# Sue1347/SMSUT-MedicalImgSegmentation

Hardware: AMD Instinct MI355X
Metric: slices/sec uganConsisTrainer step @256x256 (higher is better)
Workload: dtype f32

## Files before the change

smsut-medicalimgsegmentation_amd/csrc/conv1x1.hip:

```cpp
#include "common.h"

namespace {

typedef float f32x4 __attribute__((ext_vector_type(4)));
constexpr int TPB = 256;

__device__ __forceinline__ f32x4 mfma16(float a, float b, f32x4 c) {
  return __builtin_amdgcn_mfma_f32_16x16x4f32(a, b, c, 0, 0, 0);
}

template <int MR, int NR, bool DUAL = false, bool PS = false>
__global__ void __launch_bounds__(TPB)
conv1x1_fwd(const float* __restrict__ x, const float* __restrict__ w, float* __restrict__ y, float* __restrict__ stats,
            int64_t P, int HW, int Kdim, int Ndim, int transposed, float* __restrict__ y2 = nullptr, int split = 0,
            const float* __restrict__ x2 = nullptr, int ca = 0, int ps_w = 0) {
  constexpr int CO_T = 16 * NR;
  extern __shared__ float w_s[];
  const int tid = threadIdx.x, lane = tid & 63, wave = tid >> 6;
  const int lm = lane & 15, kq = lane >> 4;
  const int co0 = blockIdx.y * CO_T;
  const int chunks = (Kdim + 15) / 16;
  for (int u = tid; u < chunks * 4 * CO_T; u += TPB) {
    const int n = u % CO_T;
    const int kg = (u / CO_T) * 4;
    const int ng = co0 + n;
    float4 v = make_float4(0.f, 0.f, 0.f, 0.f);
    if (ng < Ndim && kg < Kdim) {
      if constexpr (PS) {
        const int cout = Ndim >> 2, tap = ng / cout;
        const float* p = w + ((size_t)tap * Kdim + kg) * cout + (ng - tap * cout);
        v.x = p[0]; v.y = p[cout]; v.z = p[2 * (size_t)cout]; v.w = p[3 * (size_t)cout];
      } else if (!transposed) {
        const float* p = w + (size_t)kg * Ndim + ng;
        v.x = p[0]; v.y = p[Ndim]; v.z = p[2 * (size_t)Ndim]; v.w = p[3 * (size_t)Ndim];
      } else {
        v = *(const float4*)(w + (size_t)ng * Kdim + kg);
      }
    }
    *(float4*)(w_s + (size_t)u * 4) = v;
  }
  __syncthreads();

  const int64_t p0 = ((int64_t)blockIdx.x * 4 + wave) * (16 * MR);
  if (p0 >= P) return;
  f32x4 acc[MR][NR];
#pragma unroll
  for (int i = 0; i < MR; ++i)
#pragma unroll
    for (int j = 0; j < NR; ++j) acc[i][j] = (f32x4){0.f, 0.f, 0.f, 0.f};
  const float* xp[MR];
  const float* xq[MR];
  bool pok[MR];
  const int sa = DUAL ? ca : Kdim;
#pragma unroll
  for (int i = 0; i < MR; ++i) {
    const int64_t p = p0 + i * 16 + lm;
    pok[i] = p < P;
    xp[i] = x + (size_t)(pok[i] ? p : 0) * sa + 4 * kq;
    xq[i] = DUAL ? x2 + (size_t)(pok[i] ? p : 0) * (Kdim - ca) + 4 * kq - ca : xp[i];
  }
  for (int c = 0; c < chunks; ++c) {
    const bool kok = c * 16 + 4 * kq < Kdim;
    const bool second = DUAL && c * 16 >= ca;
    f32x4 a[MR], b[NR];
#pragma unroll
    for (int i = 0; i < MR; ++i)
      a[i] = (pok[i] && kok) ? *(const f32x4*)((second ? xq[i] : xp[i]) + c * 16) : (f32x4){0.f, 0.f, 0.f, 0.f};
#pragma unroll
    for (int j = 0; j < NR; ++j) b[j] = *(const f32x4*)(w_s + ((size_t)(c * 4 + kq) * CO_T + j * 16 + lm) * 4);
#pragma unroll
    for (int s = 0; s < 4; ++s)
#pragma unroll
      for (int i = 0; i < MR; ++i)
#pragma unroll
        for (int j = 0; j < NR; ++j) acc[i][j] = mfma16(a[i][s], b[j][s], acc[i][j]);
  }
#pragma unroll
  for (int j = 0; j < NR; ++j) {
    const int co = co0 + j * 16 + lm;
    const bool hi = y2 && co0 + j * 16 >= split;
    float* const yo = hi ? y2 : y;
    const int os = !y2 ? Ndim : (hi ? Ndim - split : split);
    const int oc = hi ? co - split : co;
    float s1 = 0.f, s2 = 0.f;
    if constexpr (PS) {
      const int cout = Ndim >> 2, tap = (co0 + j * 16) / cout, cc = co - tap * cout;
      const int W2 = 2 * ps_w;
#pragma unroll
      for (int i = 0; i < MR; ++i)
#pragma unroll
        for (int r = 0; r < 4; ++r) {
          const int64_t p = p0 + i * 16 + 4 * kq + r;
          if (p < P && co < Ndim) {
            const int row = (int)p / ps_w;
            const int wx = (int)p - row * ps_w;
            y[((size_t)(2 * row + (tap >> 1)) * W2 + 2 * wx + (tap & 1)) * cout + cc] = acc[i][j][r];
          }
        }
      continue;
    }
#pragma unroll
    for (int i = 0; i < MR; ++i)
#pragma unroll
      for (int r = 0; r < 4; ++r) {
        const int64_t p = p0 + i * 16 + 4 * kq + r;
        if (p < P && co < Ndim) {
          const float v = acc[i][j][r];
          yo[(size_t)p * os + oc] = v;
          s1 += v; s2 += v * v;
        }
      }
    if (stats) {
      s1 += __shfl_xor(s1, 16, 64); s2 += __shfl_xor(s2, 16, 64);
      s1 += __shfl_xor(s1, 32, 64); s2 += __shfl_xor(s2, 32, 64);
      if (kq == 0 && co < Ndim) {
        const int tiles = HW / (16 * MR);
        const int64_t n_img = p0 / HW;
        const int tile = (int)((p0 % HW) / (16 * MR));
        float* o = stats + (((size_t)n_img * tiles + tile) * Ndim + co) * 2;
        o[0] = s1; o[1] = s2;
      }
    }
  }
}

#ifndef W1_UNR
#define W1_UNR 4
#endif
template <int CIT, int COT, bool PS = false>
__global__ void __launch_bounds__(TPB)
conv1x1_wgrad(const float* __restrict__ x, const float* __restrict__ gy, float* __restrict__ part, int64_t P, int Cin,
              int Cout, int64_t pix_per_split, const float* __restrict__ x2 = nullptr, int ca = 0, int ps_w = 0) {
  __shared__ float red[CIT * COT * 64 * 4];
  const int tid = threadIdx.x, lane = tid & 63, wave = tid >> 6;
  const int lm = lane & 15, kq = lane >> 4;
  const int ci0 = blockIdx.y * (16 * CIT), co0 = blockIdx.z * (16 * COT);
  const int64_t pb = (int64_t)blockIdx.x * pix_per_split;
  const int64_t pe = min(pb + pix_per_split, P);
  f32x4 acc[CIT][COT];
#pragma unroll
  for (int i = 0; i < CIT; ++i)
#pragma unroll
    for (int j = 0; j < COT; ++j) acc[i][j] = (f32x4){0.f, 0.f, 0.f, 0.f};
  bool iok[CIT], jok[COT];
#pragma unroll
  for (int i = 0; i < CIT; ++i) iok[i] = ci0 + i * 16 + lm < Cin;
#pragma unroll
  for (int j = 0; j < COT; ++j) jok[j] = co0 + j * 16 + lm < Cout;
  CatSrc xs[CIT];
#pragma unroll
  for (int i = 0; i < CIT; ++i) xs[i] = cat_src(x, x2, Cin, ca, ci0 + i * 16);
  const float* gb = gy + co0 + lm;
  [[maybe_unused]] const int cout = Cout >> 2;
  [[maybe_unused]] int ps_tap[COT], ps_cc[COT];
  if constexpr (PS) {
#pragma unroll
    for (int j = 0; j < COT; ++j) { ps_tap[j] = (co0 + j * 16) / cout; ps_cc[j] = co0 + j * 16 - ps_tap[j] * cout + lm; }
  }
  constexpr int UNR = W1_UNR;
  for (int64_t p0 = pb + 4 * wave + kq; p0 - kq < pe; p0 += 16 * UNR) {
    float a[UNR][CIT], b[UNR][COT];
#pragma unroll
    for (int u = 0; u < UNR; ++u) {
      const int64_t p = p0 + 16 * u;
      const bool ok = p < pe;
#pragma unroll
      for (int i = 0; i < CIT; ++i) a[u][i] = (ok && iok[i]) ? xs[i].p[(size_t)p * xs[i].stride + ci0 + i * 16 + lm - xs[i].coff] : 0.f;
      if constexpr (PS) {
        const int row = (int)p / ps_w;
        const int wx = (int)p - row * ps_w;
#pragma unroll
        for (int j = 0; j < COT; ++j)
          b[u][j] = (ok && jok[j]) ? gy[((size_t)(2 * row + (ps_tap[j] >> 1)) * (2 * ps_w) + 2 * wx + (ps_tap[j] & 1)) * cout + ps_cc[j]] : 0.f;
      } else {
#pragma unroll
        for (int j = 0; j < COT; ++j) b[u][j] = (ok && jok[j]) ? gb[(size_t)p * Cout + j * 16] : 0.f;
      }
    }
#pragma unroll
    for (int u = 0; u < UNR; ++u)
#pragma unroll
      for (int i = 0; i < CIT; ++i)
#pragma unroll
        for (int j = 0; j < COT; ++j) acc[i][j] = mfma16(a[u][i], b[u][j], acc[i][j]);
  }
  for (int src = 1; src < 4; ++src) {
    __syncthreads();
    if (wave == src) {
#pragma unroll
      for (int i = 0; i < CIT; ++i)
#pragma unroll
        for (int j = 0; j < COT; ++j) *(f32x4*)(red + ((size_t)(i * COT + j) * 64 + lane) * 4) = acc[i][j];
    }
    __syncthreads();
    if (wave == 0) {
#pragma unroll
      for (int i = 0; i < CIT; ++i)
#pragma unroll
        for (int j = 0; j < COT; ++j) acc[i][j] += *(const f32x4*)(red + ((size_t)(i * COT + j) * 64 + lane) * 4);
    }
  }
  if (wave == 0) {
    float* out = part + (size_t)blockIdx.x * Cin * Cout;
#pragma unroll
    for (int i = 0; i < CIT; ++i)
#pragma unroll
      for (int j = 0; j < COT; ++j) {
        const int co = co0 + j * 16 + lm;
#pragma unroll
        for (int r = 0; r < 4; ++r) {
          const int ci = ci0 + i * 16 + 4 * kq + r;
          if constexpr (PS) {
            if (ci < Cin && co < Cout) out[((size_t)ps_tap[j] * Cin + ci) * cout + ps_cc[j]] = acc[i][j][r];
          } else if (ci < Cin && co < Cout) out[(size_t)ci * Cout + co] = acc[i][j][r];
        }
      }
  }
}

__global__ void __launch_bounds__(TPB)
sum_parts(const float* __restrict__ part, float* __restrict__ out, int wsize, int splits) {
  __shared__ float4 sm[TPB];
  const int col = threadIdx.x & 15, sl = threadIdx.x >> 4;
  const int e = (blockIdx.x * 16 + col) * 4;
  float4 t0 = make_float4(0.f, 0.f, 0.f, 0.f), t1 = t0, t2 = t0, t3 = t0;
  if (e < wsize) {
    int c = sl;
    for (; c + 48 < splits; c += 64) {
      const float4 v0 = *(const float4*)(part + (size_t)c * wsize + e);
      const float4 v1 = *(const float4*)(part + (size_t)(c + 16) * wsize + e);
      const float4 v2 = *(const float4*)(part + (size_t)(c + 32) * wsize + e);
      const float4 v3 = *(const float4*)(part + (size_t)(c + 48) * wsize + e);
      t0.x += v0.x; t0.y += v0.y; t0.z += v0.z; t0.w += v0.w; t1.x += v1.x; t1.y += v1.y; t1.z += v1.z; t1.w += v1.w;
      t2.x += v2.x; t2.y += v2.y; t2.z += v2.z; t2.w += v2.w; t3.x += v3.x; t3.y += v3.y; t3.z += v3.z; t3.w += v3.w;
    }
    for (; c < splits; c += 16) {
      const float4 v = *(const float4*)(part + (size_t)c * wsize + e);
      t0.x += v.x; t0.y += v.y; t0.z += v.z; t0.w += v.w;
    }
  }
  sm[threadIdx.x] = make_float4((t0.x + t1.x) + (t2.x + t3.x), (t0.y + t1.y) + (t2.y + t3.y), (t0.z + t1.z) + (t2.z + t3.z),
                                (t0.w + t1.w) + (t2.w + t3.w));
  __syncthreads();
  if (sl == 0 && e < wsize) {
    float4 t = sm[col];
    for (int l = 1; l < 16; ++l) { const float4 v = sm[l * 16 + col]; t.x += v.x; t.y += v.y; t.z += v.z; t.w += v.w; }
    *(float4*)(out + e) = t;
  }
}

struct Plan1 { int splits; int64_t pps; };
inline Plan1 plan_wgrad1(int64_t P, int Cin, int Cout, int cit, int cot) {
  const int slabs = ((Cin + 16 * cit - 1) / (16 * cit)) * ((Cout + 16 * cot - 1) / (16 * cot));
  int64_t want = (1024 + slabs - 1) / slabs;
  const int64_t maxs = P / 256 > 0 ? P / 256 : 1;
  if (want > maxs) want = maxs;
  if (want < 1) want = 1;
  Plan1 p;
  p.pps = ((P + want - 1) / want + 15) / 16 * 16;
  p.splits = (int)((P + p.pps - 1) / p.pps);
  return p;
}


constexpr int THIN_MAX = 8;

template <int CI>
__global__ void __launch_bounds__(TPB)
thin1x1_dgrad(const float* __restrict__ gy, const float* __restrict__ w, float* __restrict__ gx, int64_t P, int CO) {
  constexpr int Q = CI / 4;
  __shared__ float wt[THIN_MAX * CI];
  for (int u = threadIdx.x; u < THIN_MAX * CI; u += TPB) {
    const int k = u / CI, ci = u % CI;
    wt[u] = k < CO ? w[ci * CO + k] : 0.f;
  }
  __syncthreads();
  const int64_t total = P * Q;
  for (int64_t i = (int64_t)blockIdx.x * TPB + threadIdx.x; i < total; i += (int64_t)gridDim.x * TPB) {
    const int c4 = (int)(i % Q);
    const int64_t px = i / Q;
    float g[THIN_MAX];
#pragma unroll
    for (int k = 0; k < THIN_MAX; ++k) g[k] = k < CO ? gy[px * CO + k] : 0.f;
    f32x4 o = {0.f, 0.f, 0.f, 0.f};
#pragma unroll
    for (int k = 0; k < THIN_MAX; ++k) o += g[k] * *(const f32x4*)(wt + k * CI + c4 * 4);
    *(f32x4*)(gx + i * 4) = o;
  }
}

template <int CI>
__global__ void __launch_bounds__(TPB)
thin1x1_wgrad(const float* __restrict__ x, const float* __restrict__ gy, float* __restrict__ part, int64_t P, int CO) {
  constexpr int Q = CI / 4;
  static_assert(Q <= 64 && (Q & (Q - 1)) == 0, "lanes sharing a channel group sit Q apart inside a wave");
  __shared__ float sm[4 * Q * 4 * THIN_MAX];
  f32x4 acc[THIN_MAX];
#pragma unroll
  for (int k = 0; k < THIN_MAX; ++k) acc[k] = (f32x4){0.f, 0.f, 0.f, 0.f};
  const int64_t total = P * Q;
  const int64_t stride = (int64_t)gridDim.x * TPB;
  auto step = [&](int64_t i) {
    const int64_t px = i / Q;
    const f32x4 xv = *(const f32x4*)(x + i * 4);
#pragma unroll
    for (int k = 0; k < THIN_MAX; ++k) {
      const float g = k < CO ? gy[px * CO + k] : 0.f;
      acc[k] += g * xv;
    }
  };
  int64_t i = (int64_t)blockIdx.x * TPB + threadIdx.x;
  for (; i + stride < total; i += 2 * stride) { step(i); step(i + stride); }
  for (; i < total; i += stride) step(i);
  for (int off = Q; off < 64; off <<= 1) {
#pragma unroll
    for (int k = 0; k < THIN_MAX; ++k)
#pragma unroll
      for (int j = 0; j < 4; ++j) acc[k][j] += __shfl_xor(acc[k][j], off, 64);
  }
  const int lane = threadIdx.x & 63, wv = threadIdx.x >> 6;
  if (lane < Q) {
#pragma unroll
    for (int k = 0; k < THIN_MAX; ++k) *(f32x4*)(sm + ((wv * Q + lane) * THIN_MAX + k) * 4) = acc[k];
  }
  __syncthreads();
  if (threadIdx.x < Q) {
    const int c4 = threadIdx.x;
#pragma unroll
    for (int k = 0; k < THIN_MAX; ++k) {
      f32x4 t = *(const f32x4*)(sm + ((0 * Q + c4) * THIN_MAX + k) * 4);
#pragma unroll
      for (int w4 = 1; w4 < 4; ++w4) t += *(const f32x4*)(sm + ((w4 * Q + c4) * THIN_MAX + k) * 4);
#pragma unroll
      for (int j = 0; j < 4; ++j) part[((size_t)blockIdx.x * CI + c4 * 4 + j) * THIN_MAX + k] = t[j];
    }
  }
}

__global__ void __launch_bounds__(TPB)
thin1x1_wsum(const float* __restrict__ part, float* __restrict__ gw, int blocks, int CI, int CO) {
  const int lane = threadIdx.x & 63;
  const int col = blockIdx.x * 4 + (threadIdx.x >> 6);
  if (col >= CI * THIN_MAX / 4) return;
  f32x4 t = {0.f, 0.f, 0.f, 0.f};
  for (int b = lane; b < blocks; b += 64) t += *(const f32x4*)(part + ((size_t)b * CI * THIN_MAX) + col * 4);
  for (int off = 1; off < 64; off <<= 1)
#pragma unroll
    for (int j = 0; j < 4; ++j) t[j] += __shfl_xor(t[j], off, 64);
  if (lane == 0) {
    const int ci = col / 2, k0 = (col & 1) * 4;
#pragma unroll
    for (int j = 0; j < 4; ++j)
      if (k0 + j < CO) gw[ci * CO + k0 + j] = t[j];
  }
}

constexpr int THIN_WGRAD_BLOCKS = 1024;

}

extern "C" {

int smsut_conv1x1_supported(int Kdim, int Ndim) { return Kdim >= 4 && (Kdim % 4) == 0 && Kdim <= 512 && Ndim >= 1; }

int smsut_conv1x1_tiles(int N, int HW, int Ndim) {
  const int64_t P = (int64_t)N * HW;
  const int mr = (P / 256 >= 512) ? 4 : 1;
  (void)Ndim;
  return (HW % (16 * mr) == 0) ? HW / (16 * mr) : 0;
}

static int conv1x1_fwd_launch(const float* x, const float* w, float* y, float* stats, int N, int HW, int Kdim, int Ndim,
                              int transposed, void* stream, float* y2, int split, const float* x2 = nullptr, int ca = 0) {
  SMSUT_REQUIRE(x && w && y && N > 0 && HW > 0 && smsut_conv1x1_supported(Kdim, Ndim));
  SMSUT_REQUIRE(!y2 || (!stats && split > 0 && split < Ndim && split % 16 == 0));
  SMSUT_REQUIRE(!x2 || (!transposed && ca > 0 && ca < Kdim && ca % 16 == 0 && (Kdim - ca) % 4 == 0));
  const int64_t P = (int64_t)N * HW;
  const int mr = (P / 256 >= 512) ? 4 : 1;
  SMSUT_REQUIRE(!stats || HW % (16 * mr) == 0);
  const int nr = Ndim <= 16 ? 1 : 2;
  const int chunks = (Kdim + 15) / 16;
  const size_t sh = (size_t)chunks * 4 * 16 * nr * 4 * sizeof(float);
  dim3 grid((unsigned)cdiv64(P, 64 * mr), (Ndim + 16 * nr - 1) / (16 * nr));
  hipStream_t st = (hipStream_t)stream;
#define LAUNCH1X1(M, R)                                                                                                      \
  do {                                                                                                                       \
    if (x2) conv1x1_fwd<M, R, true><<<grid, TPB, sh, st>>>(x, w, y, stats, P, HW, Kdim, Ndim, transposed, y2, split, x2, ca); \
    else conv1x1_fwd<M, R, false><<<grid, TPB, sh, st>>>(x, w, y, stats, P, HW, Kdim, Ndim, transposed, y2, split, nullptr, 0); \
  } while (0)
  if (mr == 4 && nr == 2) LAUNCH1X1(4, 2);
  else if (mr == 4) LAUNCH1X1(4, 1);
  else if (nr == 2) LAUNCH1X1(1, 2);
  else LAUNCH1X1(1, 1);
#undef LAUNCH1X1
  SMSUT_LAUNCH_CHECK();
  return SMSUT_OK;
}

int smsut_conv1x1_fwd(const float* x, const float* w, float* y, float* stats, int N, int HW, int Kdim, int Ndim,
                      int transposed, void* stream) {
  return conv1x1_fwd_launch(x, w, y, stats, N, HW, Kdim, Ndim, transposed, stream, nullptr, 0);
}

int smsut_conv1x1_fwd_cat(const float* xa, const float* xb, int ca, const float* w, float* y, float* stats, int N, int HW,
                          int Kdim, int Ndim, void* stream) {
  SMSUT_REQUIRE(xb);
  return conv1x1_fwd_launch(xa, w, y, stats, N, HW, Kdim, Ndim, 0, stream, nullptr, 0, xb, ca);
}

int smsut_conv1x1_fwd_split(const float* x, const float* w, float* ya, float* yb, int split, int N, int HW, int Kdim,
                            int Ndim, int transposed, void* stream) {
  SMSUT_REQUIRE(yb);
  return conv1x1_fwd_launch(x, w, ya, nullptr, N, HW, Kdim, Ndim, transposed, stream, yb, split);
}

int smsut_convT2x2_ps_supported(int Cin, int Cout) {
  return Cout == 16 && Cin <= 256 && smsut_conv1x1_supported(Cin, 4 * Cout);
}

int smsut_convT2x2_fwd_ps(const float* x, const float* w, float* y, int N, int H, int W, int Cin, int Cout, void* stream) {
  SMSUT_REQUIRE(x && w && y && N > 0 && H > 0 && W > 0 && smsut_convT2x2_ps_supported(Cin, Cout));
  const int64_t P = (int64_t)N * H * W;
  SMSUT_REQUIRE(P * 4 * Cout < (1ll << 31));
  const int Nd = 4 * Cout;
  const int mr = (P / 256 >= 512) ? 4 : 1;
  const int nr = (Nd % 64 == 0) ? 4 : 2;
  const int chunks = (Cin + 15) / 16;
  const size_t sh = (size_t)chunks * 4 * 16 * nr * 4 * sizeof(float);
  dim3 grid((unsigned)cdiv64(P, 64 * mr), Nd / (16 * nr));
  hipStream_t st = (hipStream_t)stream;
#define PS_GO(M, R) conv1x1_fwd<M, R, false, true><<<grid, TPB, sh, st>>>(x, w, y, nullptr, P, H * W, Cin, Nd, 0, nullptr, 0, nullptr, 0, W)
  if (mr == 4 && nr == 4) PS_GO(4, 4);
  else if (mr == 4) PS_GO(4, 2);
  else if (nr == 4) PS_GO(1, 4);
  else PS_GO(1, 2);
#undef PS_GO
  SMSUT_LAUNCH_CHECK();
  return SMSUT_OK;
}

int64_t smsut_convT2x2_wgrad_ps_ws(int N, int H, int W, int Cin, int Cout) {
  const int cit = Cin > 16 ? 2 : 1;
  return (int64_t)plan_wgrad1((int64_t)N * H * W, Cin, 4 * Cout, cit, 2).splits * Cin * 4 * Cout;
}

int smsut_convT2x2_wgrad_ps(const float* x, const float* gy, float* gw, float* workspace, int N, int H, int W, int Cin,
                            int Cout, void* stream) {
  SMSUT_REQUIRE(x && gy && gw && workspace && N > 0 && H > 0 && W > 0 && smsut_convT2x2_ps_supported(Cin, Cout));
  const int64_t P = (int64_t)N * H * W;
  SMSUT_REQUIRE(P * 4 * Cout < (1ll << 31));
  const int Nd = 4 * Cout;
  const int cit = Cin > 16 ? 2 : 1;
  const Plan1 p = plan_wgrad1(P, Cin, Nd, cit, 2);
  dim3 grid(p.splits, (Cin + 16 * cit - 1) / (16 * cit), Nd / 32);
  hipStream_t st = (hipStream_t)stream;
  if (cit == 2) conv1x1_wgrad<2, 2, true><<<grid, TPB, 0, st>>>(x, gy, workspace, P, Cin, Nd, p.pps, nullptr, 0, W);
  else conv1x1_wgrad<1, 2, true><<<grid, TPB, 0, st>>>(x, gy, workspace, P, Cin, Nd, p.pps, nullptr, 0, W);
  const int wsize = Cin * Nd;
  sum_parts<<<(wsize + 63) / 64, TPB, 0, st>>>(workspace, gw, wsize, p.splits);
  SMSUT_LAUNCH_CHECK();
  return SMSUT_OK;
}

int64_t smsut_conv1x1_wgrad_ws(int N, int HW, int Cin, int Cout) {
  const int cit = Cin > 16 ? 2 : 1, cot = Cout > 16 ? 2 : 1;
  return (int64_t)plan_wgrad1((int64_t)N * HW, Cin, Cout, cit, cot).splits * Cin * Cout;
}

static int conv1x1_wgrad_launch(const float* x, const float* gy, float* gw, float* workspace, int N, int HW, int Cin,
                                int Cout, void* stream, const float* x2, int ca) {
  SMSUT_REQUIRE(x && gy && gw && workspace && N > 0 && HW > 0 && Cin > 0 && Cout > 0);
  SMSUT_REQUIRE(!x2 || (ca > 0 && ca < Cin && ca % 16 == 0));
  SMSUT_REQUIRE(((int64_t)Cin * Cout) % 4 == 0);
  const int64_t P = (int64_t)N * HW;
  const int cit = Cin > 16 ? 2 : 1, cot = Cout > 16 ? 2 : 1;
  const Plan1 p = plan_wgrad1(P, Cin, Cout, cit, cot);
  dim3 grid(p.splits, (Cin + 16 * cit - 1) / (16 * cit), (Cout + 16 * cot - 1) / (16 * cot));
  hipStream_t st = (hipStream_t)stream;
  if (cit == 2 && cot == 2) conv1x1_wgrad<2, 2><<<grid, TPB, 0, st>>>(x, gy, workspace, P, Cin, Cout, p.pps, x2, ca);
  else if (cit == 2) conv1x1_wgrad<2, 1><<<grid, TPB, 0, st>>>(x, gy, workspace, P, Cin, Cout, p.pps, x2, ca);
  else if (cot == 2) conv1x1_wgrad<1, 2><<<grid, TPB, 0, st>>>(x, gy, workspace, P, Cin, Cout, p.pps, x2, ca);
  else conv1x1_wgrad<1, 1><<<grid, TPB, 0, st>>>(x, gy, workspace, P, Cin, Cout, p.pps, x2, ca);
  const int wsize = Cin * Cout;
  sum_parts<<<(wsize + 63) / 64, TPB, 0, st>>>(workspace, gw, wsize, p.splits);
  SMSUT_LAUNCH_CHECK();
  return SMSUT_OK;
}

int smsut_conv1x1_wgrad(const float* x, const float* gy, float* gw, float* workspace, int N, int HW, int Cin, int Cout,
                        void* stream) {
  return conv1x1_wgrad_launch(x, gy, gw, workspace, N, HW, Cin, Cout, stream, nullptr, 0);
}

int smsut_conv1x1_wgrad_cat(const float* xa, const float* xb, int ca, const float* gy, float* gw, float* workspace, int N,
                            int HW, int Cin, int Cout, void* stream) {
  SMSUT_REQUIRE(xb);
  return conv1x1_wgrad_launch(xa, gy, gw, workspace, N, HW, Cin, Cout, stream, xb, ca);
}

int smsut_conv1x1_thin_supported(int Cin, int Cout) {
  return (Cin == 8 || Cin == 16 || Cin == 32 || Cin == 64) && Cout >= 1 && Cout <= THIN_MAX;
}

int smsut_conv1x1_thin_dgrad(const float* gy, const float* w, float* gx, int N, int HW, int Cin, int Cout, void* stream) {
  SMSUT_REQUIRE(gy && w && gx && N > 0 && HW > 0 && smsut_conv1x1_thin_supported(Cin, Cout));
  const int64_t P = (int64_t)N * HW;
  hipStream_t st = (hipStream_t)stream;
  const int grid = ew_grid(P * (Cin / 4));
  switch (Cin) {
    case 8: thin1x1_dgrad<8><<<grid, TPB, 0, st>>>(gy, w, gx, P, Cout); break;
    case 16: thin1x1_dgrad<16><<<grid, TPB, 0, st>>>(gy, w, gx, P, Cout); break;
    case 32: thin1x1_dgrad<32><<<grid, TPB, 0, st>>>(gy, w, gx, P, Cout); break;
    default: thin1x1_dgrad<64><<<grid, TPB, 0, st>>>(gy, w, gx, P, Cout); break;
  }
  SMSUT_LAUNCH_CHECK();
  return SMSUT_OK;
}

int64_t smsut_conv1x1_thin_wgrad_ws(int Cin) { return (int64_t)THIN_WGRAD_BLOCKS * Cin * THIN_MAX; }

int smsut_conv1x1_thin_wgrad(const float* x, const float* gy, float* gw, float* workspace, int N, int HW, int Cin,
                             int Cout, void* stream) {
  SMSUT_REQUIRE(x && gy && gw && workspace && N > 0 && HW > 0 && smsut_conv1x1_thin_supported(Cin, Cout));
  const int64_t P = (int64_t)N * HW;
  hipStream_t st = (hipStream_t)stream;
  int blocks = (int)cdiv64(P * (Cin / 4), 2 * TPB);
  if (blocks > THIN_WGRAD_BLOCKS) blocks = THIN_WGRAD_BLOCKS;
  switch (Cin) {
    case 8: thin1x1_wgrad<8><<<blocks, TPB, 0, st>>>(x, gy, workspace, P, Cout); break;
    case 16: thin1x1_wgrad<16><<<blocks, TPB, 0, st>>>(x, gy, workspace, P, Cout); break;
    case 32: thin1x1_wgrad<32><<<blocks, TPB, 0, st>>>(x, gy, workspace, P, Cout); break;
    default: thin1x1_wgrad<64><<<blocks, TPB, 0, st>>>(x, gy, workspace, P, Cout); break;
  }
  thin1x1_wsum<<<(Cin * THIN_MAX / 4 + 3) / 4, TPB, 0, st>>>(workspace, gw, blocks, Cin, Cout);
  SMSUT_LAUNCH_CHECK();
  return SMSUT_OK;
}

}
```

Baseline: 830.9.

## Make 1x1 conv forward persistent with prefetched inputs and LDS-staged vector stores

Turns the 1x1 conv forward kernel into a persistent grid. Each workgroup stages the weights into LDS once and then walks many pixel tiles, double-buffering the next group of input chunks in registers so the loads overlap the MFMA work. Output tiles are transposed through a small per-wave LDS exchange so they can be written as 16-byte vector stores instead of scalar strided stores. The weight staging loop is also unrolled. In exchange the kernel adds register pressure from the prefetch buffers and more template variants, and the occupancy-based grid cap may leave some CUs underused.

```diff
diff --git a/smsut-medicalimgsegmentation_amd/csrc/conv1x1.hip b/smsut-medicalimgsegmentation_amd/csrc/conv1x1.hip
--- a/smsut-medicalimgsegmentation_amd/csrc/conv1x1.hip
+++ b/smsut-medicalimgsegmentation_amd/csrc/conv1x1.hip
@@ -1,4 +1,5 @@
 #include "common.h"
+#include <type_traits>
 
 namespace {
 
@@ -9,119 +10,190 @@
   return __builtin_amdgcn_mfma_f32_16x16x4f32(a, b, c, 0, 0, 0);
 }
 
-template <int MR, int NR, bool DUAL = false, bool PS = false>
+#define FENCE1() do { asm volatile("" ::: "memory"); __builtin_amdgcn_sched_barrier(0); } while (0)
+
+#ifndef FWD1_WGS_PER_CU_MR1
+#define FWD1_WGS_PER_CU_MR1 4
+#endif
+#ifndef FWD1_WGS_PER_CU_MR4
+#define FWD1_WGS_PER_CU_MR4 2
+#endif
+constexpr int FWD1_AHEAD = 4;
+constexpr int FWD1_STAGE_UNR = 4;
+constexpr int XCH_STRIDE = 20;
+constexpr int XCH_FLOATS = 4 * 16 * XCH_STRIDE;
+
+template <int MR, int NR, int G, bool DUAL = false, bool PS = false>
 __global__ void __launch_bounds__(TPB)
 conv1x1_fwd(const float* __restrict__ x, const float* __restrict__ w, float* __restrict__ y, float* __restrict__ stats,
-            int64_t P, int HW, int Kdim, int Ndim, int transposed, float* __restrict__ y2 = nullptr, int split = 0,
+            int64_t P, int HW, int Kdim, int Ndim, int transposed, int xchg, float* __restrict__ y2 = nullptr, int split = 0,
             const float* __restrict__ x2 = nullptr, int ca = 0, int ps_w = 0) {
   constexpr int CO_T = 16 * NR;
-  extern __shared__ float w_s[];
+  extern __shared__ __attribute__((aligned(16))) float w_s[];
   const int tid = threadIdx.x, lane = tid & 63, wave = tid >> 6;
   const int lm = lane & 15, kq = lane >> 4;
   const int co0 = blockIdx.y * CO_T;
   const int chunks = (Kdim + 15) / 16;
-  for (int u = tid; u < chunks * 4 * CO_T; u += TPB) {
-    const int n = u % CO_T;
-    const int kg = (u / CO_T) * 4;
-    const int ng = co0 + n;
-    float4 v = make_float4(0.f, 0.f, 0.f, 0.f);
-    if (ng < Ndim && kg < Kdim) {
-      if constexpr (PS) {
-        const int cout = Ndim >> 2, tap = ng / cout;
-        const float* p = w + ((size_t)tap * Kdim + kg) * cout + (ng - tap * cout);
-        v.x = p[0]; v.y = p[cout]; v.z = p[2 * (size_t)cout]; v.w = p[3 * (size_t)cout];
-      } else if (!transposed) {
-        const float* p = w + (size_t)kg * Ndim + ng;
-        v.x = p[0]; v.y = p[Ndim]; v.z = p[2 * (size_t)Ndim]; v.w = p[3 * (size_t)Ndim];
-      } else {
-        v = *(const float4*)(w + (size_t)ng * Kdim + kg);
+  const int64_t ntiles = (P + 16 * MR - 1) / (16 * MR);
+  const int64_t tstride = (int64_t)gridDim.x * 4;
+  int64_t t = (int64_t)blockIdx.x * 4 + wave;
+  const int ngroups = (chunks + G - 1) / G;
+  int g = 0;
+  const int sa = DUAL ? ca : Kdim;
+  auto load = [&](f32x4 (&a)[G][MR], int64_t tile, int grp) {
+#pragma unroll
+    for (int i = 0; i < MR; ++i) {
+      const int64_t p = tile * (16 * MR) + i * 16 + lm;
+      const size_t pc = p < P ? (size_t)p : 0;
+      const float* xa = x + pc * sa;
+      [[maybe_unused]] const float* xb = DUAL ? x2 + pc * (Kdim - ca) : xa;
+#pragma unroll
+      for (int cc = 0; cc < G; ++cc) {
+        const int k = (grp * G + cc) * 16 + 4 * kq;
+        const bool second = DUAL && (grp * G + cc) * 16 >= ca;
+        const int off = k < Kdim ? (second ? k - ca : k) : 0;
+        a[cc][i] = *(const f32x4*)((second ? xb : xa) + off);
       }
     }
-    *(float4*)(w_s + (size_t)u * 4) = v;
-  }
+  };
+  f32x4 a0[G][MR], a1[G][MR];
+
+  const int units = chunks * 4 * CO_T;
+  auto stage = [&](auto tr_c) {
+    constexpr bool TR = decltype(tr_c)::value;
+    for (int u0 = tid; u0 < units; u0 += TPB * FWD1_STAGE_UNR) {
+      float4 v[FWD1_STAGE_UNR];
+#pragma unroll
+      for (int s = 0; s < FWD1_STAGE_UNR; ++s) {
+        const int u = u0 + s * TPB;
+        const int n = u % CO_T;
+        const int kg = (u / CO_T) * 4;
+        const int ng = co0 + n;
+        const bool ok = u < units && ng < Ndim && kg < Kdim;
+        if constexpr (PS) {
+          const int cout = Ndim >> 2, tap = ng / cout;
+          const float* p = ok ? w + ((size_t)tap * Kdim + kg) * cout + (ng - tap * cout) : w;
+          const size_t sw = ok ? cout : 0;
+          v[s] = make_float4(p[0], p[sw], p[2 * sw], p[3 * sw]);
+        } else if constexpr (!TR) {
+          const float* p = ok ? w + (size_t)kg * Ndim + ng : w;
+          const size_t sw = ok ? Ndim : 0;
+          v[s] = make_float4(p[0], p[sw], p[2 * sw], p[3 * sw]);
+        } else {
+          v[s] = *(const float4*)(ok ? w + (size_t)ng * Kdim + kg : w);
+        }
+        if (!ok) v[s] = make_float4(0.f, 0.f, 0.f, 0.f);
+      }
+#pragma unroll
+      for (int s = 0; s < FWD1_STAGE_UNR; ++s)
+        if (u0 + s * TPB < units) *(float4*)(w_s + (size_t)(u0 + s * TPB) * 4) = v[s];
+    }
+  };
+  if (PS || !transposed) stage(std::false_type{});
+  else stage(std::true_type{});
   __syncthreads();
 
-  const int64_t p0 = ((int64_t)blockIdx.x * 4 + wave) * (16 * MR);
-  if (p0 >= P) return;
+  if (t >= ntiles) return;
+  load(a0, t, 0);
   f32x4 acc[MR][NR];
 #pragma unroll
   for (int i = 0; i < MR; ++i)
 #pragma unroll
     for (int j = 0; j < NR; ++j) acc[i][j] = (f32x4){0.f, 0.f, 0.f, 0.f};
-  const float* xp[MR];
-  const float* xq[MR];
-  bool pok[MR];
-  const int sa = DUAL ? ca : Kdim;
-#pragma unroll
-  for (int i = 0; i < MR; ++i) {
-    const int64_t p = p0 + i * 16 + lm;
-    pok[i] = p < P;
-    xp[i] = x + (size_t)(pok[i] ? p : 0) * sa + 4 * kq;
-    xq[i] = DUAL ? x2 + (size_t)(pok[i] ? p : 0) * (Kdim - ca) + 4 * kq - ca : xp[i];
-  }
-  for (int c = 0; c < chunks; ++c) {
-    const bool kok = c * 16 + 4 * kq < Kdim;
-    const bool second = DUAL && c * 16 >= ca;
-    f32x4 a[MR], b[NR];
-#pragma unroll
-    for (int i = 0; i < MR; ++i)
-      a[i] = (pok[i] && kok) ? *(const f32x4*)((second ? xq[i] : xp[i]) + c * 16) : (f32x4){0.f, 0.f, 0.f, 0.f};
-#pragma unroll
-    for (int j = 0; j < NR; ++j) b[j] = *(const f32x4*)(w_s + ((size_t)(c * 4 + kq) * CO_T + j * 16 + lm) * 4);
-#pragma unroll
-    for (int s = 0; s < 4; ++s)
-#pragma unroll
-      for (int i = 0; i < MR; ++i)
-#pragma unroll
-        for (int j = 0; j < NR; ++j) acc[i][j] = mfma16(a[i][s], b[j][s], acc[i][j]);
-  }
-#pragma unroll
-  for (int j = 0; j < NR; ++j) {
-    const int co = co0 + j * 16 + lm;
-    const bool hi = y2 && co0 + j * 16 >= split;
-    float* const yo = hi ? y2 : y;
-    const int os = !y2 ? Ndim : (hi ? Ndim - split : split);
-    const int oc = hi ? co - split : co;
-    float s1 = 0.f, s2 = 0.f;
-    if constexpr (PS) {
-      const int cout = Ndim >> 2, tap = (co0 + j * 16) / cout, cc = co - tap * cout;
-      const int W2 = 2 * ps_w;
-#pragma unroll
-      for (int i = 0; i < MR; ++i)
-#pragma unroll
-        for (int r = 0; r < 4; ++r) {
-          const int64_t p = p0 + i * 16 + 4 * kq + r;
-          if (p < P && co < Ndim) {
+
+  auto unit = [&](f32x4 (&cur)[G][MR], f32x4 (&nxt)[G][MR]) -> bool {
+    int64_t tn = t;
+    int gn = g + 1;
+    if (gn == ngroups) { gn = 0; tn = t + tstride; }
+    if (tn < ntiles) load(nxt, tn, gn);
+    FENCE1();
+    const int64_t p0 = t * (16 * MR);
+#pragma unroll
+    for (int cc = 0; cc < G; ++cc) {
+      const int c = g * G + cc;
+      if (c < chunks) {
+        const bool kok = c * 16 + 4 * kq < Kdim;
+        f32x4 a[MR], b[NR];
+#pragma unroll
+        for (int i = 0; i < MR; ++i) a[i] = (kok && p0 + i * 16 + lm < P) ? cur[cc][i] : (f32x4){0.f, 0.f, 0.f, 0.f};
+#pragma unroll
+        for (int j = 0; j < NR; ++j) b[j] = *(const f32x4*)(w_s + ((size_t)(c * 4 + kq) * CO_T + j * 16 + lm) * 4);
+#pragma unroll
+        for (int s = 0; s < 4; ++s)
+#pragma unroll
+          for (int i = 0; i < MR; ++i)
+#pragma unroll
+            for (int j = 0; j < NR; ++j) acc[i][j] = mfma16(a[i][s], b[j][s], acc[i][j]);
+      }
+    }
+    if (gn == 0) {
+      float* const xs = w_s + (size_t)chunks * 4 * CO_T * 4 + wave * (16 * XCH_STRIDE);
+      const int pp = lane >> 2, cq = (lane & 3) * 4;
+#pragma unroll
+      for (int j = 0; j < NR; ++j) {
+        const int co = co0 + j * 16 + lm;
+        const bool hi = y2 && co0 + j * 16 >= split;
+        float* const yo = hi ? y2 : y;
+        const int os = !y2 ? Ndim : (hi ? Ndim - split : split);
+        float s1 = 0.f, s2 = 0.f;
+        [[maybe_unused]] const int cout = Ndim >> 2, tap = PS ? (co0 + j * 16) / cout : 0, W2 = 2 * ps_w;
+        auto opix = [&](int64_t p) -> size_t {
+          if constexpr (PS) {
             const int row = (int)p / ps_w;
             const int wx = (int)p - row * ps_w;
-            y[((size_t)(2 * row + (tap >> 1)) * W2 + 2 * wx + (tap & 1)) * cout + cc] = acc[i][j][r];
+            return (size_t)(2 * row + (tap >> 1)) * W2 + 2 * wx + (tap & 1);
+          } else {
+            return (size_t)p;
+          }
+        };
+        const int ost = PS ? cout : os;
+        const int ocb = PS ? co0 + j * 16 - tap * cout : (hi ? co0 + j * 16 - split : co0 + j * 16);
+        const bool vec = xchg && (ost & 3) == 0 && co0 + j * 16 + 16 <= Ndim && ((uintptr_t)yo & 15) == 0;
+#pragma unroll
+        for (int i = 0; i < MR; ++i) {
+          if (vec) {
+#pragma unroll
+            for (int r = 0; r < 4; ++r) xs[(4 * kq + r) * XCH_STRIDE + lm] = acc[i][j][r];
+            __builtin_amdgcn_wave_barrier();
+            const f32x4 v = *(const f32x4*)(xs + pp * XCH_STRIDE + cq);
+            __builtin_amdgcn_wave_barrier();
+            const int64_t p = p0 + i * 16 + pp;
+            if (p < P) *(f32x4*)(yo + opix(p) * ost + ocb + cq) = v;
+          } else {
+#pragma unroll
+            for (int r = 0; r < 4; ++r) {
+              const int64_t p = p0 + i * 16 + 4 * kq + r;
+              if (p < P && co < Ndim) yo[opix(p) * ost + ocb + lm] = acc[i][j][r];
+            }
+          }
+          if (!PS && stats) {
+#pragma unroll
+            for (int r = 0; r < 4; ++r) {
+              const float v = acc[i][j][r];
+              float q = v * v;
+              asm("" : "+v"(q));
+              if (p0 + i * 16 + 4 * kq + r < P && co < Ndim) { s1 += v; s2 += q; }
+            }
+          }
+          acc[i][j] = (f32x4){0.f, 0.f, 0.f, 0.f};
+        }
+        if (!PS && stats) {
+          s1 += __shfl_xor(s1, 16, 64); s2 += __shfl_xor(s2, 16, 64);
+          s1 += __shfl_xor(s1, 32, 64); s2 += __shfl_xor(s2, 32, 64);
+          if (kq == 0 && co < Ndim) {
+            const int tiles = HW / (16 * MR);
+            const int64_t n_img = p0 / HW;
+            const int tile = (int)((p0 % HW) / (16 * MR));
+            float* o = stats + (((size_t)n_img * tiles + tile) * Ndim + co) * 2;
+            o[0] = s1; o[1] = s2;
           }
         }
-      continue;
-    }
-#pragma unroll
-    for (int i = 0; i < MR; ++i)
-#pragma unroll
-      for (int r = 0; r < 4; ++r) {
-        const int64_t p = p0 + i * 16 + 4 * kq + r;
-        if (p < P && co < Ndim) {
-          const float v = acc[i][j][r];
-          yo[(size_t)p * os + oc] = v;
-          s1 += v; s2 += v * v;
-        }
       }
-    if (stats) {
-      s1 += __shfl_xor(s1, 16, 64); s2 += __shfl_xor(s2, 16, 64);
-      s1 += __shfl_xor(s1, 32, 64); s2 += __shfl_xor(s2, 32, 64);
-      if (kq == 0 && co < Ndim) {
-        const int tiles = HW / (16 * MR);
-        const int64_t n_img = p0 / HW;
-        const int tile = (int)((p0 % HW) / (16 * MR));
-        float* o = stats + (((size_t)n_img * tiles + tile) * Ndim + co) * 2;
-        o[0] = s1; o[1] = s2;
-      }
-    }
-  }
+    }
+    t = tn; g = gn;
+    return t < ntiles;
+  };
+  while (unit(a0, a1) && unit(a1, a0)) {}
 }
 
 #ifndef W1_UNR
@@ -249,6 +321,20 @@
   }
 }
 
+struct Geo1 { unsigned wgs; int g; size_t lds; int xchg; };
+inline Geo1 fwd1_geometry(int64_t P, int mr, int nr, int chunks, int slabs) {
+  Geo1 o;
+  const int64_t wg_tiles = cdiv64(cdiv64(P, 16 * mr), 4);
+  const int cap = (mr == 4 ? FWD1_WGS_PER_CU_MR4 : FWD1_WGS_PER_CU_MR1) * 256 / slabs;
+  o.wgs = (unsigned)(wg_tiles < cap ? wg_tiles : (cap > 1 ? cap : 1));
+  if (mr == 4) o.g = chunks >= 4 ? 2 : 1;
+  else o.g = chunks == 1 ? 1 : (chunks == 2 ? 2 : FWD1_AHEAD);
+  o.lds = (size_t)chunks * 4 * 16 * nr * 4 * sizeof(float);
+  o.xchg = o.lds + XCH_FLOATS * sizeof(float) <= 65536;
+  if (o.xchg) o.lds += XCH_FLOATS * sizeof(float);
+  return o;
+}
+
 struct Plan1 { int splits; int64_t pps; };
 inline Plan1 plan_wgrad1(int64_t P, int Cin, int Cout, int cit, int cot) {
   const int slabs = ((Cin + 16 * cit - 1) / (16 * cit)) * ((Cout + 16 * cot - 1) / (16 * cot));
@@ -380,19 +466,27 @@
   SMSUT_REQUIRE(!stats || HW % (16 * mr) == 0);
   const int nr = Ndim <= 16 ? 1 : 2;
   const int chunks = (Kdim + 15) / 16;
-  const size_t sh = (size_t)chunks * 4 * 16 * nr * 4 * sizeof(float);
-  dim3 grid((unsigned)cdiv64(P, 64 * mr), (Ndim + 16 * nr - 1) / (16 * nr));
+  const int slabs = (Ndim + 16 * nr - 1) / (16 * nr);
+  const Geo1 geo = fwd1_geometry(P, mr, nr, chunks, slabs);
+  dim3 grid(geo.wgs, slabs);
   hipStream_t st = (hipStream_t)stream;
+#define GO1X1(M, R, G)                                                                                                                 \
+  do {                                                                                                                                 \
+    if (x2) conv1x1_fwd<M, R, G, true><<<grid, TPB, geo.lds, st>>>(x, w, y, stats, P, HW, Kdim, Ndim, transposed, geo.xchg, y2, split, x2, ca); \
+    else conv1x1_fwd<M, R, G, false><<<grid, TPB, geo.lds, st>>>(x, w, y, stats, P, HW, Kdim, Ndim, transposed, geo.xchg, y2, split, nullptr, 0); \
+  } while (0)
 #define LAUNCH1X1(M, R)                                                                                                      \
   do {                                                                                                                       \
-    if (x2) conv1x1_fwd<M, R, true><<<grid, TPB, sh, st>>>(x, w, y, stats, P, HW, Kdim, Ndim, transposed, y2, split, x2, ca); \
-    else conv1x1_fwd<M, R, false><<<grid, TPB, sh, st>>>(x, w, y, stats, P, HW, Kdim, Ndim, transposed, y2, split, nullptr, 0); \
+    if (geo.g == 1) GO1X1(M, R, 1);                                                                                          \
+    else if (geo.g == 2) GO1X1(M, R, 2);                                                                                     \
+    else GO1X1(M, R, FWD1_AHEAD);                                                                                            \
   } while (0)
   if (mr == 4 && nr == 2) LAUNCH1X1(4, 2);
   else if (mr == 4) LAUNCH1X1(4, 1);
   else if (nr == 2) LAUNCH1X1(1, 2);
   else LAUNCH1X1(1, 1);
 #undef LAUNCH1X1
+#undef GO1X1
   SMSUT_LAUNCH_CHECK();
   return SMSUT_OK;
 }
@@ -426,15 +520,22 @@
   const int mr = (P / 256 >= 512) ? 4 : 1;
   const int nr = (Nd % 64 == 0) ? 4 : 2;
   const int chunks = (Cin + 15) / 16;
-  const size_t sh = (size_t)chunks * 4 * 16 * nr * 4 * sizeof(float);
-  dim3 grid((unsigned)cdiv64(P, 64 * mr), Nd / (16 * nr));
+  const Geo1 geo = fwd1_geometry(P, mr, nr, chunks, Nd / (16 * nr));
+  dim3 grid(geo.wgs, Nd / (16 * nr));
   hipStream_t st = (hipStream_t)stream;
-#define PS_GO(M, R) conv1x1_fwd<M, R, false, true><<<grid, TPB, sh, st>>>(x, w, y, nullptr, P, H * W, Cin, Nd, 0, nullptr, 0, nullptr, 0, W)
+#define PS_GO1(M, R, G) conv1x1_fwd<M, R, G, false, true><<<grid, TPB, geo.lds, st>>>(x, w, y, nullptr, P, H * W, Cin, Nd, 0, geo.xchg, nullptr, 0, nullptr, 0, W)
+#define PS_GO(M, R)                         \
+  do {                                      \
+    if (geo.g == 1) PS_GO1(M, R, 1);        \
+    else if (geo.g == 2) PS_GO1(M, R, 2);   \
+    else PS_GO1(M, R, FWD1_AHEAD);          \
+  } while (0)
   if (mr == 4 && nr == 4) PS_GO(4, 4);
   else if (mr == 4) PS_GO(4, 2);
   else if (nr == 4) PS_GO(1, 4);
   else PS_GO(1, 2);
 #undef PS_GO
+#undef PS_GO1
   SMSUT_LAUNCH_CHECK();
   return SMSUT_OK;
 }
```

New measurement: 831.2 (median of 2 runs). About the same (+0.0%).
